# researchaccelerator-hub/distributed-crawler

Hardware: AMD Instinct MI355X
Metric: posts/sec (whole node) synthetic feed (higher is better)
Workload: dtype uint8; 1 GPU; model=telegram-crawl 1k-channels x 10k-posts per GPU (BASELINE config #2, weak-scaled), global_batch=1250000, seq_len=0, platform=telegram, parallelism=dp1, channels_per_gpu=1000, posts_per_channel=10000, chunk_posts=1250000, new_discoveries=998486, sink=pinned, pinned=True, max_comments_per_post=3

## Files before the change

### crawler_amd/ops/csrc/common.h

```cpp
#pragma once

#include <hip/hip_runtime.h>
#include <stdint.h>

#define WAVE 64
#define DEV __device__ __forceinline__

typedef unsigned int __attribute__((aligned(1))) u32_unal;
#ifndef CRAWL_NT_STORES
#define CRAWL_NT_STORES 0
#endif
DEV void nt_store_u32(unsigned char* p, unsigned v) {
#if CRAWL_NT_STORES
  __builtin_nontemporal_store(v, (u32_unal*)p);
#else
  __builtin_memcpy(p, &v, 4);
#endif
}
DEV void nt_store_u8(unsigned char* p, unsigned char v) {
#if CRAWL_NT_STORES
  __builtin_nontemporal_store(v, p);
#else
  *p = v;
#endif
}

namespace crawl {

DEV int lane_id() { return threadIdx.x & (WAVE - 1); }
DEV int wave_id() { return threadIdx.x >> 6; }


DEV bool is_ascii_letter(uint8_t c) {
  return (c >= 'a' && c <= 'z') || (c >= 'A' && c <= 'Z');
}
DEV bool is_word_char(uint8_t c) {
  return is_ascii_letter(c) || (c >= '0' && c <= '9') || c == '_';
}
DEV uint8_t to_lower(uint8_t c) {
  return (c >= 'A' && c <= 'Z') ? (c + 32) : c;
}

DEV int u16_units_of_byte(uint8_t b) {
  if (b < 0x80) return 1;
  if (b < 0xC0) return 0;
  if (b < 0xF0) return 1;
  return 2;
}

__device__ const uint8_t ESC_CLS[256] = {
    0x06, 0x06, 0x06, 0x06, 0x06, 0x06, 0x06, 0x06, 0x06, 0x02, 0x02, 0x06, 0x06, 0x02, 0x06, 0x06,
    0x06, 0x06, 0x06, 0x06, 0x06, 0x06, 0x06, 0x06, 0x06, 0x06, 0x06, 0x06, 0x06, 0x06, 0x06, 0x06,
    0x01, 0x01, 0x02, 0x01, 0x01, 0x01, 0x06, 0x01, 0x01, 0x01, 0x01, 0x01, 0x01, 0x01, 0x01, 0x01,
    0x01, 0x01, 0x01, 0x01, 0x01, 0x01, 0x01, 0x01, 0x01, 0x01, 0x01, 0x01, 0x06, 0x01, 0x06, 0x01,
    0x01, 0x01, 0x01, 0x01, 0x01, 0x01, 0x01, 0x01, 0x01, 0x01, 0x01, 0x01, 0x01, 0x01, 0x01, 0x01,
    0x01, 0x01, 0x01, 0x01, 0x01, 0x01, 0x01, 0x01, 0x01, 0x01, 0x01, 0x01, 0x02, 0x01, 0x01, 0x01,
    0x01, 0x01, 0x01, 0x01, 0x01, 0x01, 0x01, 0x01, 0x01, 0x01, 0x01, 0x01, 0x01, 0x01, 0x01, 0x01,
    0x01, 0x01, 0x01, 0x01, 0x01, 0x01, 0x01, 0x01, 0x01, 0x01, 0x01, 0x01, 0x01, 0x01, 0x01, 0x01,
    0xFF, 0x01, 0x01, 0x01, 0x01, 0x01, 0x01, 0x01, 0x01, 0x01, 0x01, 0x01, 0x01, 0x01, 0x01, 0x01,
    0x01, 0x01, 0x01, 0x01, 0x01, 0x01, 0x01, 0x01, 0x01, 0x01, 0x01, 0x01, 0x01, 0x01, 0x01, 0x01,
    0x01, 0x01, 0x01, 0x01, 0x01, 0x01, 0x01, 0x01, 0xFF, 0xFF, 0x01, 0x01, 0x01, 0x01, 0x01, 0x01,
    0x01, 0x01, 0x01, 0x01, 0x01, 0x01, 0x01, 0x01, 0x01, 0x01, 0x01, 0x01, 0x01, 0x01, 0x01, 0x01,
    0x01, 0x01, 0x01, 0x01, 0x01, 0x01, 0x01, 0x01, 0x01, 0x01, 0x01, 0x01, 0x01, 0x01, 0x01, 0x01,
    0x01, 0x01, 0x01, 0x01, 0x01, 0x01, 0x01, 0x01, 0x01, 0x01, 0x01, 0x01, 0x01, 0x01, 0x01, 0x01,
    0x01, 0x01, 0xFF, 0x01, 0x01, 0x01, 0x01, 0x01, 0x01, 0x01, 0x01, 0x01, 0x01, 0x01, 0x01, 0x01,
    0x01, 0x01, 0x01, 0x01, 0x01, 0x01, 0x01, 0x01, 0x01, 0x01, 0x01, 0x01, 0x01, 0x01, 0x01, 0x01,
};

DEV int escape_len_at(const uint8_t* s, int n, int p) {
  uint8_t c = s[p];
  uint8_t v = ESC_CLS[c];
  if (v != 0xFF) return v;
  if (c == 0xE2) {
    if (p + 2 < n && s[p + 1] == 0x80 &&
        (s[p + 2] == 0xA8 || s[p + 2] == 0xA9))
      return 6;
    return 1;
  }
  if (c == 0x80) {
    if (p >= 1 && s[p - 1] == 0xE2 && p + 1 < n &&
        (s[p + 1] == 0xA8 || s[p + 1] == 0xA9))
      return 0;
    return 1;
  }
  if (p >= 2 && s[p - 2] == 0xE2 && s[p - 1] == 0x80) return 0;
  return 1;
}

DEV const char* HEXD() { return "0123456789abcdef"; }

DEV int escape_write_at(const uint8_t* s, int n, int p, uint8_t* out) {
  uint8_t c = s[p];
  switch (c) {
    case '"':  out[0] = '\\'; out[1] = '"';  return 2;
    case '\\': out[0] = '\\'; out[1] = '\\'; return 2;
    case '\n': out[0] = '\\'; out[1] = 'n';  return 2;
    case '\r': out[0] = '\\'; out[1] = 'r';  return 2;
    case '\t': out[0] = '\\'; out[1] = 't';  return 2;
    default: break;
  }
  if (c < 0x20 || c == '<' || c == '>' || c == '&') {
    out[0] = '\\'; out[1] = 'u'; out[2] = '0'; out[3] = '0';
    out[4] = HEXD()[c >> 4]; out[5] = HEXD()[c & 15];
    return 6;
  }
  if (c == 0xE2 && p + 2 < n && s[p + 1] == 0x80 &&
      (s[p + 2] == 0xA8 || s[p + 2] == 0xA9)) {
    out[0] = '\\'; out[1] = 'u'; out[2] = '2'; out[3] = '0'; out[4] = '2';
    out[5] = (s[p + 2] == 0xA8) ? '8' : '9';
    return 6;
  }
  if (escape_len_at(s, n, p) == 0) return 0;
  out[0] = c;
  return 1;
}


DEV int wave_prefix_excl(int v) {
  int lane = lane_id();
  for (int d = 1; d < WAVE; d <<= 1) {
    int up = __shfl_up(v, d);
    if (lane >= d) v += up;
  }
  return __shfl_up(v, 1) * (lane > 0 ? 1 : 0);
}

DEV int wave_sum(int v) {
  for (int d = WAVE / 2; d > 0; d >>= 1) v += __shfl_down(v, d);
  return __shfl(v, 0);
}


DEV int u64_dec_len(uint64_t v) {
  if (v < 10ULL) return 1;
  if (v < 100ULL) return 2;
  if (v < 1000ULL) return 3;
  if (v < 10000ULL) return 4;
  if (v < 100000ULL) return 5;
  if (v < 1000000ULL) return 6;
  if (v < 10000000ULL) return 7;
  if (v < 100000000ULL) return 8;
  if (v < 1000000000ULL) return 9;
  if (v < 10000000000ULL) return 10;
  if (v < 100000000000ULL) return 11;
  if (v < 1000000000000ULL) return 12;
  if (v < 10000000000000ULL) return 13;
  if (v < 100000000000000ULL) return 14;
  if (v < 1000000000000000ULL) return 15;
  if (v < 10000000000000000ULL) return 16;
  if (v < 100000000000000000ULL) return 17;
  if (v < 1000000000000000000ULL) return 18;
  if (v < 10000000000000000000ULL) return 19;
  return 20;
}
DEV int i64_dec_len(int64_t v) {
  return (v < 0) ? 1 + u64_dec_len((uint64_t)(-v)) : u64_dec_len((uint64_t)v);
}

DEV void rfc3339_write(uint8_t* out, int cur, long long secs) {
  long long days = secs / 86400;
  long long rem = secs % 86400;
  if (rem < 0) { rem += 86400; days -= 1; }
  int hh = (int)(rem / 3600), mm = (int)((rem % 3600) / 60),
      ss = (int)(rem % 60);
  long long z = days + 719468;
  long long era = (z >= 0 ? z : z - 146096) / 146097;
  long long doe = z - era * 146097;
  long long yoe = (doe - doe / 1460 + doe / 36524 - doe / 146096) / 365;
  long long y = yoe + era * 400;
  long long doy = doe - (365 * yoe + yoe / 4 - yoe / 100);
  long long mp = (5 * doy + 2) / 153;
  long long d = doy - (153 * mp + 2) / 5 + 1;
  long long m = mp + (mp < 10 ? 3 : -9);
  y += (m <= 2);
  int yy = (int)y, mo = (int)m, dd = (int)d;
  auto pk = [](int a, int b, int c, int e) {
    return (unsigned)a | ((unsigned)b << 8) | ((unsigned)c << 16) |
           ((unsigned)e << 24);
  };
  unsigned w0 = pk('0' + (yy / 1000) % 10, '0' + (yy / 100) % 10,
                   '0' + (yy / 10) % 10, '0' + yy % 10);
  unsigned w1 = pk('-', '0' + mo / 10, '0' + mo % 10, '-');
  unsigned w2 = pk('0' + dd / 10, '0' + dd % 10, 'T', '0' + hh / 10);
  unsigned w3 = pk('0' + hh % 10, ':', '0' + mm / 10, '0' + mm % 10);
  unsigned w4 = pk(':', '0' + ss / 10, '0' + ss % 10, 'Z');
  int lane = lane_id();
  if (lane < 5) {
    unsigned v = w0;
    if (lane == 1) v = w1;
    else if (lane == 2) v = w2;
    else if (lane == 3) v = w3;
    else if (lane == 4) v = w4;
    nt_store_u32(out + cur + 4 * lane, v);
  }
}

#define LIT(e, s)                                              \
  do {                                                         \
    if ((int)sizeof(s) - 1 <= 4)                               \
      (e).template lit_small<(int)sizeof(s) - 1>(s);           \
    else                                                       \
      (e).raw((const unsigned char*)(s), (int)sizeof(s) - 1);  \
  } while (0)

template <bool W>
struct JsonEmit {
  uint8_t* out;
  int cur;
  const uint8_t* lds;

  DEV void lds_lit(int off, int n) {
    if (W) {
      const uint8_t* s = lds + off;
      int lane = lane_id();
      int nw = n >> 2;
      for (int k = lane; k < nw; k += WAVE) {
        unsigned w;
        __builtin_memcpy(&w, s + 4 * k, 4);
        nt_store_u32(out + cur + 4 * k, w);
      }
      for (int j = (nw << 2) + lane; j < n; j += WAVE)
        nt_store_u8(out + cur + j, s[j]);
    }
    cur += n;
  }

  template <int N, int M>
  DEV void lit_small(const char (&str)[M]) {
    if (W && lane_id() == 0) {
      if (N == 1) {
        out[cur] = (unsigned char)str[0];
      } else if (N == 2) {
        unsigned short v = (unsigned short)((unsigned char)str[0] |
                                            ((unsigned char)str[1] << 8));
        __builtin_memcpy(out + cur, &v, 2);
      } else {
        unsigned v = (unsigned)(unsigned char)str[0] |
                     ((unsigned)(unsigned char)str[1] << 8) |
                     ((N > 2 ? (unsigned)(unsigned char)str[2] : 0u) << 16) |
                     ((N > 3 ? (unsigned)(unsigned char)str[3] : 0u) << 24);
        if (N == 4)
          __builtin_memcpy(out + cur, &v, 4);
        else {
          __builtin_memcpy(out + cur, &v, 2);
          out[cur + 2] = (unsigned char)str[2];
        }
      }
    }
    cur += N;
  }

  DEV void raw(const uint8_t* s, int n) {
    if (W) {
      int lane = lane_id();
      int nw = n >> 2;
      for (int k = lane; k < nw; k += WAVE) {
        unsigned w;
        __builtin_memcpy(&w, s + 4 * k, 4);
        nt_store_u32(out + cur + 4 * k, w);
      }
      for (int j = (nw << 2) + lane; j < n; j += WAVE)
        nt_store_u8(out + cur + j, s[j]);
    }
    cur += n;
  }

  static DEV bool swar_special(unsigned w) {
    unsigned hz;
    unsigned nonascii = w & 0x80808080u;
    unsigned lt20 = (w - 0x20202020u) & ~w & 0x80808080u;
    if (lt20) return true;
    hz = ((w ^ 0x22222222u) - 0x01010101u) & ~(w ^ 0x22222222u);
    hz |= ((w ^ 0x5C5C5C5Cu) - 0x01010101u) & ~(w ^ 0x5C5C5C5Cu);
    hz |= ((w ^ 0x3C3C3C3Cu) - 0x01010101u) & ~(w ^ 0x3C3C3C3Cu);
    hz |= ((w ^ 0x3E3E3E3Eu) - 0x01010101u) & ~(w ^ 0x3E3E3E3Eu);
    hz |= ((w ^ 0x26262626u) - 0x01010101u) & ~(w ^ 0x26262626u);
    if (hz & 0x80808080u) return true;
    if (nonascii) {
      unsigned e2 = ((w ^ 0xE2E2E2E2u) - 0x01010101u) & ~(w ^ 0xE2E2E2E2u);
      if (e2 & 0x80808080u) return true;
    }
    return false;
  }

  DEV void esc(const uint8_t* s, int n) {
    int lane = lane_id();
    int start = 0;
    while (start < n) {
      if (start + 4 * WAVE <= n) {
        bool risk = (start >= 1 && s[start - 1] == 0xE2) ||
                    (start >= 2 && s[start - 2] == 0xE2 &&
                     s[start - 1] == 0x80);
        if (!risk) {
          unsigned w;
          __builtin_memcpy(&w, s + start + 4 * lane, 4);
          if (__ballot(swar_special(w)) == 0) {
            if (W)
              nt_store_u32(out + cur + 4 * lane, w);
            cur += 4 * WAVE;
            start += 4 * WAVE;
            continue;
          }
        }
      }
      esc_stripe(s, n, start, lane);
      start += WAVE;
    }
  }

  DEV void esc_stripe(const uint8_t* s, int n, int start, int lane) {
    {
      int p = start + lane;
      int span = n - start;
      if (span > WAVE) span = WAVE;
      int el = (p < n) ? escape_len_at(s, n, p) : 0;
      unsigned long long dirty = __ballot(p < n && el != 1);
      if (dirty == 0) {
        if (W && p < n) nt_store_u8(out + cur + p - start, s[p]);
        cur += span;
        return;
      }
      if (W) {
        int off = wave_prefix_excl(el);
        if (p < n && el > 0) {
          escape_write_at(s, n, p, out + cur + off);
        }
      }
      cur += wave_sum(el);
    }
  }

  DEV void u64(unsigned long long v) {
    static const unsigned long long POW10[20] = {
        1ULL, 10ULL, 100ULL, 1000ULL, 10000ULL, 100000ULL, 1000000ULL,
        10000000ULL, 100000000ULL, 1000000000ULL, 10000000000ULL,
        100000000000ULL, 1000000000000ULL, 10000000000000ULL,
        100000000000000ULL, 1000000000000000ULL, 10000000000000000ULL,
        100000000000000000ULL, 1000000000000000000ULL,
        10000000000000000000ULL};
    int n = u64_dec_len(v);
    if (W) {
      int lane = lane_id();
      if (lane < n) {
        unsigned d;
        if (v <= 0xFFFFFFFFULL)
          d = ((unsigned)v / (unsigned)POW10[lane]) % 10u;
        else
          d = (unsigned)((v / POW10[lane]) % 10ULL);
        nt_store_u8(out + cur + n - 1 - lane, (uint8_t)('0' + d));
      }
    }
    cur += n;
  }
  DEV void i64(long long v) {
    if (v < 0) { LIT(*this, "-"); u64((unsigned long long)(-v)); }
    else u64((unsigned long long)v);
  }

  DEV void rfc3339(long long secs) {
    if (W) rfc3339_write(out, cur, secs);
    cur += 20;
  }
};

DEV uint64_t fnv1a64(const uint8_t* s, int n) {
  uint64_t h = 1469598103934665603ULL;
  for (int i = 0; i < n; ++i) {
    h ^= s[i];
    h *= 1099511628211ULL;
  }
  return h;
}

}
```

### crawler_amd/ops/csrc/gen_lits.py

```python
#!/usr/bin/env python3
import os
import re

SRC = os.path.join(os.path.dirname(os.path.abspath(__file__)),
                   "parse_encode.hip")
OUT = os.path.join(os.path.dirname(os.path.abspath(__file__)),
                   "tg_lits.h")


def c_unescape_len(lit: str) -> int:
    i = 0
    n = 0
    while i < len(lit):
        if lit[i] == "\\":
            i += 2
        else:
            i += 1
        n += 1
    return n


def main():
    src = open(SRC).read()
    start = src.index("DEV int emit_line")
    end = src.index("\n}", start)
    body = src[start:end]
    lits = re.findall(r'LIT\(e,\s*((?:"(?:[^"\\]|\\.)*"\s*)+)\)', body)
    strings = []
    for raw in lits:
        segs = re.findall(r'"((?:[^"\\]|\\.)*)"', raw)
        strings.append("".join(segs))
    seen = {}
    order = []
    for s in strings:
        if c_unescape_len(s) >= 5 and s not in seen:
            seen[s] = f"TGL_{len(order)}"
            order.append(s)

    lines = ["// GENERATED by gen_lits.py — do not edit by hand.",
             "// LDS literal pool for parse_encode.hip's emit_line.",
             "#pragma once", "", "namespace crawl {", ""]
    lines.append("#define TG_LIT_STRS(X) \\")
    for s in order:
        lines.append(f'  X({seen[s]}, "{s}") \\')
    lines.append("")
    lines.append("enum TgLitId {")
    lines.append("#define TG_ID(name, str) name##_id,")
    lines.append("TG_LIT_STRS(TG_ID)")
    lines.append("#undef TG_ID")
    lines.append("  TG_NLITS")
    lines.append("};")
    lines.append("")
    lines.append("constexpr int tg_lit_lens[] = {")
    lines.append("#define TG_LEN(name, str) (int)sizeof(str) - 1,")
    lines.append("TG_LIT_STRS(TG_LEN)")
    lines.append("#undef TG_LEN")
    lines.append("};")
    lines.append("""
constexpr int tg_lit_off(int id) {
  int o = 0;
  for (int k = 0; k < id; ++k) o += tg_lit_lens[k];
  return o;
}
constexpr int TG_POOL_BYTES = tg_lit_off(TG_NLITS);

template <int N> struct TgCharArr { char v[N]; };
constexpr TgCharArr<TG_POOL_BYTES> tg_make_pool() {
  TgCharArr<TG_POOL_BYTES> a{};
  int o = 0;
#define TG_CP(name, str) \\
  for (int k = 0; k < (int)sizeof(str) - 1; ++k) a.v[o++] = (str)[k];
TG_LIT_STRS(TG_CP)
#undef TG_CP
  return a;
}
__device__ constexpr TgCharArr<TG_POOL_BYTES> tg_lit_pool = tg_make_pool();

// call-site macro: emit pooled literal `name` from the LDS copy
#define TGLIT(e, name) \\
  (e).lds_lit(tg_lit_off(name##_id), tg_lit_lens[name##_id])
""")
    lines.append("}  // namespace crawl")
    open(OUT, "w").write("\n".join(lines) + "\n")
    print(f"{len(order)} pooled literals, {sum(c_unescape_len(s) for s in order)} bytes")

    def repl(m):
        segs = re.findall(r'"((?:[^"\\]|\\.)*)"', m.group(1))
        s = "".join(segs)
        if s in seen:
            return f"TGLIT(e, {seen[s]})"
        return m.group(0)

    new_body = re.sub(r'LIT\(e,\s*((?:"(?:[^"\\]|\\.)*"\s*)+)\)', repl,
                      body)
    open(SRC, "w").write(src[:start] + new_body + src[end:])
    n = len(re.findall(r"TGLIT\(", new_body))
    print(f"rewrote {n} call sites in emit_line")


if __name__ == "__main__":
    main()
```

### crawler_amd/ops/csrc/parse_encode.hip

```cpp

#include "common.h"
#include "tg_lits.h"
#include "views.h"

namespace crawl {

#define MAX_LINKS 8
#define TG_STAGE_BYTES 3968

struct BatchView {
  BatchView_FIELDS_0(VIEW_MEMBER)
  int created_len;
  BatchView_FIELDS_1(VIEW_MEMBER)
  int capture_len;
  int n;
  int skip_media;
  long min_post_date;
  BatchView_FIELDS_2(VIEW_MEMBER)
};

struct LinkOut {
  LinkOut_FIELDS(VIEW_MEMBER)
};


DEV void utf16_to_bytes(const unsigned char* s, int n, int off16, int len16,
                        int* out_start, int* out_end) {
  int lane = lane_id();
  int run = 0;
  int start = -1, end = -1;
  const int t1 = off16, t2 = off16 + len16;
  for (int base = 0; base < n; base += WAVE) {
    int p = base + lane;
    int u = (p < n) ? u16_units_of_byte(s[p]) : 0;
    int pre = run + wave_prefix_excl(u);
    bool boundary = (p < n) && u > 0;
    unsigned long long m1 = __ballot(boundary && pre == t1);
    unsigned long long m2 = __ballot(boundary && pre == t2);
    if (start < 0 && m1) start = base + __ffsll(m1) - 1;
    if (end < 0 && m2) end = base + __ffsll(m2) - 1;
    run += wave_sum(u);
    if (end >= 0) break;
  }
  if (start < 0) { *out_start = 0; *out_end = 0; return; }
  *out_start = start;
  *out_end = (end >= 0) ? end : n;
}


DEV bool is_reserved_path(const unsigned char* name, int n) {
  const char* tbl[10] = {"joinchat", "addlist", "addstickers", "addtheme",
                         "setlanguage", "share", "proxy", "socks", "login",
                         "confirm"};
  const int lens[10] = {8, 7, 11, 8, 11, 5, 5, 5, 5, 7};
  for (int k = 0; k < 10; ++k) {
    if (lens[k] != n) continue;
    bool eq = true;
    for (int j = 0; j < n; ++j) eq &= (name[j] == (unsigned char)tbl[k][j]);
    if (eq) return true;
  }
  return false;
}

DEV int match_name_at(const unsigned char* s, int hi, int q,
                      unsigned char* name, bool* reserved) {
  *reserved = false;
  if (q >= hi || !is_ascii_letter(s[q])) return 0;
  int len = 0;
  while (len < 32 && q + len < hi && is_word_char(s[q + len])) ++len;
  if (len < 5) return 0;
  for (int j = 0; j < len; ++j) name[j] = to_lower(s[q + j]);
  *reserved = is_reserved_path(name, len);
  return len;
}

DEV int find_tme(const unsigned char* s, int from, int hi, int lane) {
  for (int base = from; base + 5 <= hi; base += WAVE) {
    int p = base + lane;
    bool m = (p + 5 <= hi) && s[p] == 't' && s[p + 1] == '.' &&
             s[p + 2] == 'm' && s[p + 3] == 'e' && s[p + 4] == '/';
    unsigned long long bal = __ballot(m);
    if (bal) return base + __ffsll(bal) - 1;
  }
  return -1;
}

DEV int find_username(const unsigned char* s, int lo, int hi, int lane,
                      unsigned char* name) {
  for (int base = lo; base < hi; base += WAVE) {
    int p = base + lane;
    bool m = false;
    if (p < hi && p + 5 <= hi && is_ascii_letter(s[p])) {
      m = is_word_char(s[p + 1]) && is_word_char(s[p + 2]) &&
          is_word_char(s[p + 3]) && is_word_char(s[p + 4]);
    }
    unsigned long long bal = __ballot(m);
    if (bal) {
      int q = base + __ffsll(bal) - 1;
      int len = 0;
      while (len < 32 && q + len < hi && is_word_char(s[q + len])) ++len;
      for (int j = 0; j < len; ++j) name[j] = to_lower(s[q + j]);
      return len;
    }
  }
  return 0;
}

struct LinkList {
  unsigned char* names;
  unsigned char* lens;
  unsigned char* srcs;
  unsigned long long* hashes;
  int cnt;

  DEV void add(const unsigned char* name, int len, int src, int lane) {
    for (int k = 0; k < cnt; ++k) {
      if (lens[k] != (unsigned char)len) continue;
      bool eq = true;
      for (int j = 0; j < len; ++j) eq &= (names[k * 32 + j] == name[j]);
      if (eq) return;
    }
    if (cnt >= MAX_LINKS) return;
    if (lane == 0) {
      for (int j = 0; j < len; ++j) names[cnt * 32 + j] = name[j];
      lens[cnt] = (unsigned char)len;
      srcs[cnt] = (unsigned char)src;
      hashes[cnt] = fnv1a64(name, len);
    }
    ++cnt;
  }
};

DEV void extract_links(const BatchView& B, int i, LinkList& L, int lane) {
  int ct = B.content_type[i];
  if (ct > 6) return;
  const unsigned char* text = B.pool + B.text_off[i];
  const int tn = B.text_len[i];
  unsigned char name[32];

  const int e0 = B.ent_off[i], ec = B.ent_cnt[i];
  for (int e = e0; e < e0 + ec; ++e) {
    const int* row = B.entities + (long)e * 5;
    int etype = row[0];
    if (etype == 1) {
      const unsigned char* url = B.pool + row[3];
      int un = row[4];
      for (int from = 0;;) {
        int p = find_tme(url, from, un, lane);
        if (p < 0) break;
        bool rsv;
        int len = match_name_at(url, un, p + 5, name, &rsv);
        if (len) {
          if (!rsv) L.add(name, len, 1, lane);
          break;
        }
        from = p + 1;
      }
    } else {
      int lo, hi;
      utf16_to_bytes(text, tn, row[1], row[2], &lo, &hi);
      if (!(lo < hi && hi <= tn)) continue;
      if (etype == 0) {
        int len = find_username(text, lo, hi, lane, name);
        if (len) L.add(name, len, 0, lane);
      } else {
        for (int from = lo;;) {
          int p = find_tme(text, from, hi, lane);
          if (p < 0) break;
          bool rsv;
          int len = match_name_at(text, hi, p + 5, name, &rsv);
          if (len) {
            if (!rsv) L.add(name, len, 2, lane);
            break;
          }
          from = p + 1;
        }
      }
    }
  }

  int cursor = 0;
  int from = 0;
  while (true) {
    int p = find_tme(text, from, tn, lane);
    if (p < 0) break;
    from = p + 1;
    if (p < cursor) continue;
    bool rsv;
    int len = match_name_at(text, tn, p + 5, name, &rsv);
    if (len) {
      if (!rsv) L.add(name, len, 3, lane);
      cursor = p + 5 + len;
      from = cursor;
    }
  }
}


template <bool W>
struct Emit : JsonEmit<W> {
  DEV void qesc(const unsigned char* s, int n) {
    LIT(*this, "\"");
    this->esc(s, n);
    LIT(*this, "\"");
  }
};

struct StagedTabs {
  const unsigned char* emoji_pool;
  const int* emoji_off;
  const int* emoji_len;
  const unsigned char* created;
  const unsigned char* capture;
  const unsigned char* ctname_pool;
  const int* ctname_off;
  const int* ctname_len;
};

template <bool W, bool STAGED>
DEV int emit_line(const BatchView& B, int i, unsigned char* out,
                  LinkList& L, const unsigned char* lds_lits,
                  unsigned char* lds_stage, const StagedTabs* T) {
  const int lane = lane_id();
  Emit<W> e{};
  e.out = out;
  e.cur = 0;
  e.lds = lds_lits;
  const int c = B.channel_idx[i];
  const unsigned char* user = B.pool + B.ch_user_off[c];
  const int user_n = B.ch_user_len[c];
  const unsigned char* title = B.pool + B.ch_title_off[c];
  const int title_n = B.ch_title_len[c];
  const long pub_id = B.msg_id[i] >> 20;
  const int ct = B.content_type[i];
  const int ncom = B.com_cnt[i];
  const bool has_user = user_n > 0;
  const long chat_id_v = B.chat_id[i];
  const int media_album = B.media_album_id[i];
  const int date_v = B.date[i];
  const int views_v = B.views[i];
  const int forwards_v = B.forwards[i];
  const int ch_member_v = B.ch_member[c];
  const int ch_postcount_v = B.ch_postcount[c];
  const int ch_totalviews_v = B.ch_totalviews[c];
  const int flags_v = B.flags[i];
  const int com0_v = B.com_off[i];
  const int react0_v = B.react_off[i];
  const int reactc_v = B.react_cnt[i];
  const int poster_off_v = B.poster_off[i];
  const int poster_len_v = B.poster_len[i];
  const int text_off_v = B.text_off[i];
  const int text_len_v = B.text_len[i];
  const int aux_off_v = B.aux_off[i];
  const int aux_len_v = B.aux_len[i];
  const int ctname_off_v = B.ctname_off[ct];
  const int ctname_len_v = B.ctname_len[ct];
  const unsigned char* desc_p;
  int desc_n;
  if (ct == 0 || ct == 1 || ct == 2 || ct == 4 || ct == 14) {
    desc_p = B.pool + text_off_v;
    desc_n = text_len_v;
  } else if (ct == 3 || ct == 9 || ct == 10 || ct == 11) {
    desc_p = B.pool + aux_off_v;
    desc_n = aux_len_v;
  } else {
    desc_p = nullptr;
    desc_n = 0;
  }
  const unsigned char* poster_p = B.pool + poster_off_v;
  const int* re_src = B.react_emoji + react0_v;
  const int* rcnt_src = B.react_count + react0_v;
  const unsigned char* lnames_src = L.names;
  const unsigned char* llens_src = L.lens;
  if (STAGED) {
    int stage_o = 0;
    auto staged = [&](const unsigned char* ptr,
                      int n) -> const unsigned char* {
      unsigned char* dst = lds_stage + stage_o;
      stage_o += n;
      for (int j = lane; j < n; j += WAVE) dst[j] = ptr[j];
      return dst;
    };
    user = staged(user, user_n);
    title = staged(title, title_n);
    poster_p = staged(poster_p, poster_len_v);
    desc_p = staged(desc_p, desc_n);
    lnames_src = staged(L.names, L.cnt * 32);
    llens_src = staged(L.lens, L.cnt);
    stage_o = (stage_o + 3) & ~3;
    int* s_re = (int*)(lds_stage + stage_o);
    stage_o += reactc_v * 4;
    int* s_rc = (int*)(lds_stage + stage_o);
    stage_o += reactc_v * 4;
    for (int j = lane; j < reactc_v; j += WAVE) {
      s_re[j] = B.react_emoji[react0_v + j];
      s_rc[j] = B.react_count[react0_v + j];
    }
    re_src = s_re;
    rcnt_src = s_rc;
  }
  const unsigned char* emoji_pool_s = STAGED ? T->emoji_pool : B.emoji_pool;
  const int* emoji_off_s = STAGED ? T->emoji_off : B.emoji_off;
  const int* emoji_len_s = STAGED ? T->emoji_len : B.emoji_len;
  const unsigned char* created_s = STAGED ? T->created : B.created_str;
  const unsigned char* capture_s = STAGED ? T->capture : B.capture_str;
  const unsigned char* ctpool_s = STAGED ? T->ctname_pool : B.ctname_pool;

  auto post_link = [&]() {
    if (!has_user) { LIT(e, "\"\""); return; }
    TGLIT(e, TGL_0);
    e.esc(user, user_n);
    LIT(e, "/");
    e.i64(pub_id);
    if (media_album != 0) TGLIT(e, TGL_1);
    LIT(e, "\"");
  };

  TGLIT(e, TGL_2);
  post_link();
  TGLIT(e, TGL_3);
  e.i64(chat_id_v);
  TGLIT(e, TGL_4);
  e.i64(pub_id);
  LIT(e, "-");
  e.esc(user, user_n);
  TGLIT(e, TGL_5);
  post_link();
  TGLIT(e, TGL_6);
  e.rfc3339(date_v);
  TGLIT(e, TGL_7);
  e.raw(created_s, B.created_len);
  TGLIT(e, TGL_8);
  e.i64(views_v);
  TGLIT(e, TGL_9);
  e.i64(views_v);
  TGLIT(e, TGL_10);
  e.i64(forwards_v);
  TGLIT(e, TGL_11);
  e.i64(ncom);
  TGLIT(e, TGL_12);
  e.qesc(title, title_n);
  TGLIT(e, TGL_13);
  e.i64(chat_id_v);
  TGLIT(e, TGL_14);
  e.qesc(title, title_n);
  TGLIT(e, TGL_15);
  e.i64(ch_member_v);
  TGLIT(e, TGL_16);
  e.i64(ch_postcount_v);
  TGLIT(e, TGL_17);
  e.i64(ch_totalviews_v);
  TGLIT(e, TGL_18);
  e.esc(user, user_n);
  TGLIT(e, TGL_19);
  e.esc(user, user_n);
  TGLIT(e, TGL_20);
  e.qesc(desc_p, desc_n);
  TGLIT(e, TGL_21);
  e.raw(ctpool_s + (STAGED ? T->ctname_off[ct] : ctname_off_v),
        STAGED ? T->ctname_len[ct] : ctname_len_v);
  TGLIT(e, TGL_22);
  e.i64(forwards_v);
  TGLIT(e, TGL_23);
  e.i64(ncom);
  TGLIT(e, TGL_17);
  e.i64(views_v);
  TGLIT(e, TGL_24);
  TGLIT(e, TGL_25);
  if ((ct == 3 || ct == 8) && (flags_v & 2)) {
    LIT(e, "AgAD");
    e.i64(pub_id);
    LIT(e, "v");
  }
  TGLIT(e, TGL_26);
  {
    const int c0 = com0_v;
    for (int k = 0; k < ncom; ++k) {
      if (k) LIT(e, ",");
      const int cc = c0 + k;
      TGLIT(e, TGL_27);
      e.qesc(B.pool + B.com_text_off[cc], B.com_text_len[cc]);
      TGLIT(e, TGL_28);
      const int r0 = B.com_react_off[cc], rc = B.com_react_cnt[cc];
      for (int r = 0; r < rc; ++r) {
        if (r) LIT(e, ",");
        int em = B.react_emoji[r0 + r];
        LIT(e, "\"");
        e.raw(emoji_pool_s + emoji_off_s[em], emoji_len_s[em]);
        LIT(e, "\":");
        e.i64(B.react_count[r0 + r]);
      }
      TGLIT(e, TGL_29);
      e.i64(B.com_views[cc]);
      TGLIT(e, TGL_30);
      e.i64(B.com_replies[cc]);
      TGLIT(e, TGL_31);
      e.qesc(B.pool + B.com_handle_off[cc], B.com_handle_len[cc]);
      LIT(e, "}");
    }
  }
  TGLIT(e, TGL_32);
  {
    const int rc = reactc_v;
    for (int r = 0; r < rc; ++r) {
      if (r) LIT(e, ",");
      int em = re_src[r];
      LIT(e, "\"");
      e.raw(emoji_pool_s + emoji_off_s[em], emoji_len_s[em]);
      LIT(e, "\":");
      e.i64(rcnt_src[r]);
    }
  }
  TGLIT(e, TGL_33);
  for (int k = 0; k < L.cnt; ++k) {
    if (k) LIT(e, ",");
    LIT(e, "\"");
    e.raw(lnames_src + k * 32, llens_src[k]);
    LIT(e, "\"");
  }
  TGLIT(e, TGL_34);
  e.raw(capture_s, B.capture_len);
  TGLIT(e, TGL_35);
  e.qesc(poster_p, poster_len_v);
  LIT(e, "}\n");
  return e.cur;
}


DEV LinkList links_of(const LinkOut& LO, int i, int cnt) {
  return LinkList{LO.name + (size_t)i * MAX_LINKS * 32,
                  LO.name_len + (size_t)i * MAX_LINKS,
                  LO.src + (size_t)i * MAX_LINKS,
                  LO.hash + (size_t)i * MAX_LINKS, cnt};
}

__global__ void __launch_bounds__(256, 6)
measure_extract_kernel(BatchView B, LinkOut LO, int* __restrict__ line_len) {
  __shared__ unsigned char s_lits[TG_POOL_BYTES];
  __shared__ unsigned char s_ln[4][MAX_LINKS * 32];
  __shared__ unsigned char s_ll[4][MAX_LINKS];
  __shared__ unsigned char s_ls[4][MAX_LINKS];
  __shared__ unsigned long long s_lh[4][MAX_LINKS];
  for (int t = threadIdx.x; t < TG_POOL_BYTES; t += blockDim.x)
    s_lits[t] = (unsigned char)tg_lit_pool.v[t];
  __syncthreads();
  const int lane = lane_id();
  const int wave = wave_id();
  const int waves_per_grid = gridDim.x * 4;
  for (int i = blockIdx.x * 4 + wave; i < B.n; i += waves_per_grid) {
    if ((long)B.date[i] < B.min_post_date) {
      if (lane == 0) { line_len[i] = 0; LO.cnt[i] = 0; }
      continue;
    }
    LinkList L{&s_ln[wave][0], &s_ll[wave][0], &s_ls[wave][0],
               &s_lh[wave][0], 0};
    extract_links(B, i, L, lane);
    int len = emit_line<false, false>(B, i, nullptr, L, s_lits,
                                     nullptr, nullptr);
    const int nb = L.cnt * 32;
    unsigned char* gname = LO.name + (size_t)i * MAX_LINKS * 32;
    for (int j = lane; j < nb; j += WAVE) gname[j] = s_ln[wave][j];
    if (lane < L.cnt) {
      LO.name_len[(size_t)i * MAX_LINKS + lane] = s_ll[wave][lane];
      LO.src[(size_t)i * MAX_LINKS + lane] = s_ls[wave][lane];
      LO.hash[(size_t)i * MAX_LINKS + lane] = s_lh[wave][lane];
    }
    if (lane == 0) {
      line_len[i] = len;
      LO.cnt[i] = L.cnt;
    }
  }
}

__global__ void __launch_bounds__(256, 4)
write_kernel(BatchView B, LinkOut LO, const long* __restrict__ line_off,
             const int* __restrict__ line_len, unsigned char* __restrict__ out) {
  __shared__ unsigned char s_lits[TG_POOL_BYTES];
  for (int t = threadIdx.x; t < TG_POOL_BYTES; t += blockDim.x)
    s_lits[t] = (unsigned char)tg_lit_pool.v[t];
  __syncthreads();
  const int lane = lane_id();
  const int wave = wave_id();
  const int waves_per_grid = gridDim.x * 4;
  for (int i = blockIdx.x * 4 + wave; i < B.n; i += waves_per_grid) {
    if (line_len[i] == 0) continue;
    LinkList L = links_of(LO, i, LO.cnt[i]);
    emit_line<true, false>(B, i, out + line_off[i], L, s_lits, nullptr,
                           nullptr);
  }
}

#define TG_EMOJI_POOL_CAP 512
#define TG_EMOJI_CAP 64
#define TG_TS_CAP 64
#define TG_CTNAME_POOL_CAP 512
#define TG_CTNAME_CAP 32

__global__ void __launch_bounds__(256, 4)
write_staged_kernel(BatchView B, LinkOut LO, const long* __restrict__ line_off,
                    const int* __restrict__ line_len,
                    unsigned char* __restrict__ out,
                    int n_emoji, int emoji_pool_bytes,
                    int n_ctnames, int ctname_pool_bytes) {
  __shared__ unsigned char s_lits[TG_POOL_BYTES];
  __shared__ unsigned char s_stage[4][TG_STAGE_BYTES];
  __shared__ unsigned char s_emoji_pool[TG_EMOJI_POOL_CAP];
  __shared__ int s_emoji_off[TG_EMOJI_CAP];
  __shared__ int s_emoji_len[TG_EMOJI_CAP];
  __shared__ unsigned char s_created[TG_TS_CAP];
  __shared__ unsigned char s_capture[TG_TS_CAP];
  __shared__ unsigned char s_ctpool[TG_CTNAME_POOL_CAP];
  __shared__ int s_ctoff[TG_CTNAME_CAP];
  __shared__ int s_ctlen[TG_CTNAME_CAP];
  for (int t = threadIdx.x; t < TG_POOL_BYTES; t += blockDim.x)
    s_lits[t] = (unsigned char)tg_lit_pool.v[t];
  for (int t = threadIdx.x; t < emoji_pool_bytes; t += blockDim.x)
    s_emoji_pool[t] = B.emoji_pool[t];
  for (int t = threadIdx.x; t < n_emoji; t += blockDim.x) {
    s_emoji_off[t] = B.emoji_off[t];
    s_emoji_len[t] = B.emoji_len[t];
  }
  for (int t = threadIdx.x; t < B.created_len; t += blockDim.x)
    s_created[t] = B.created_str[t];
  for (int t = threadIdx.x; t < B.capture_len; t += blockDim.x)
    s_capture[t] = B.capture_str[t];
  for (int t = threadIdx.x; t < ctname_pool_bytes; t += blockDim.x)
    s_ctpool[t] = B.ctname_pool[t];
  for (int t = threadIdx.x; t < n_ctnames; t += blockDim.x) {
    s_ctoff[t] = B.ctname_off[t];
    s_ctlen[t] = B.ctname_len[t];
  }
  __syncthreads();
  StagedTabs T{s_emoji_pool, s_emoji_off, s_emoji_len, s_created,
               s_capture, s_ctpool, s_ctoff, s_ctlen};
  const int lane = lane_id();
  const int wave = wave_id();
  const int waves_per_grid = gridDim.x * 4;
  for (int i = blockIdx.x * 4 + wave; i < B.n; i += waves_per_grid) {
    if (line_len[i] == 0) continue;
    LinkList L = links_of(LO, i, LO.cnt[i]);
    emit_line<true, true>(B, i, out + line_off[i], L, s_lits,
                          &s_stage[wave][0], &T);
  }
}


#define LDS_LINE_BYTES 3072

DEV void copy_line(const unsigned char* src, unsigned char* dst, int n,
                   int lane);

__global__ void __launch_bounds__(256)
write_lds_kernel(BatchView B, LinkOut LO, const long* __restrict__ line_off,
                 const int* __restrict__ line_len, unsigned char* __restrict__ out) {
  __shared__ unsigned char lbuf[4][LDS_LINE_BYTES];
  __shared__ unsigned char s_lits[TG_POOL_BYTES];
  for (int t = threadIdx.x; t < TG_POOL_BYTES; t += blockDim.x)
    s_lits[t] = (unsigned char)tg_lit_pool.v[t];
  __syncthreads();
  const int lane = lane_id();
  const int wave = wave_id();
  const int waves_per_grid = gridDim.x * 4;
  for (int i = blockIdx.x * 4 + wave; i < B.n; i += waves_per_grid) {
    const int len = line_len[i];
    if (len == 0) continue;
    LinkList L = links_of(LO, i, LO.cnt[i]);
    if (len > LDS_LINE_BYTES) {
      emit_line<true, false>(B, i, out + line_off[i], L, s_lits,
                             nullptr, nullptr);
      continue;
    }
    emit_line<true, false>(B, i, &lbuf[wave][0], L, s_lits, nullptr,
                           nullptr);
    copy_line(&lbuf[wave][0], out + line_off[i], len, lane);
  }
}


__global__ void __launch_bounds__(256)
write_scratch_kernel(BatchView B, LinkOut LO, unsigned char* __restrict__ scratch,
                     long stride, int* __restrict__ line_len, int* __restrict__ overflow) {
  __shared__ unsigned char s_lits[TG_POOL_BYTES];
  for (int t = threadIdx.x; t < TG_POOL_BYTES; t += blockDim.x)
    s_lits[t] = (unsigned char)tg_lit_pool.v[t];
  __syncthreads();
  const int lane = lane_id();
  const int wave = wave_id();
  const int waves_per_grid = gridDim.x * 4;
  for (int i = blockIdx.x * 4 + wave; i < B.n; i += waves_per_grid) {
    if ((long)B.date[i] < B.min_post_date) {
      if (lane == 0) { line_len[i] = 0; LO.cnt[i] = 0; }
      continue;
    }
    LinkList L = links_of(LO, i, 0);
    extract_links(B, i, L, lane);
    int len = emit_line<true, false>(B, i, scratch + (size_t)i * stride, L,
                                     s_lits, nullptr, nullptr);
    if (lane == 0) {
      line_len[i] = len;
      LO.cnt[i] = L.cnt;
      if (len > stride) atomicMax(overflow, len);
    }
  }
}

DEV void copy_line(const unsigned char* src, unsigned char* dst, int n,
                   int lane) {
  int h = (int)((4 - ((unsigned long)(size_t)dst & 3)) & 3);
  if (h > n) h = n;
  if (lane == 0)
    for (int j = 0; j < h; ++j) dst[j] = src[j];
  const unsigned char* s = src + h;
  unsigned char* d = dst + h;
  int rem = n - h;
  int nw = rem >> 2;
  int sh = (int)((unsigned long)(size_t)s & 3);
  const unsigned int* sw = (const unsigned int*)(s - sh);
  for (int k = lane; k < nw; k += WAVE) {
    unsigned int w0 = sw[k];
    unsigned int v;
    if (sh) {
      unsigned int w1 = sw[k + 1];
      v = (unsigned int)((((unsigned long long)w1 << 32) | w0) >> (8 * sh));
    } else {
      v = w0;
    }
    ((unsigned int*)d)[k] = v;
  }
  if (lane == 0)
    for (int j = h + (nw << 2); j < n; ++j) dst[j] = src[j];
}

__global__ void __launch_bounds__(256)
compact_kernel(const unsigned char* scratch, long stride,
               const long* line_off, const int* line_len,
               unsigned char* out, int n) {
  const int lane = lane_id();
  const int wave = wave_id();
  const int waves_per_grid = gridDim.x * 4;
  for (int i = blockIdx.x * 4 + wave; i < n; i += waves_per_grid) {
    int len = line_len[i];
    if (len == 0) continue;
    copy_line(scratch + (size_t)i * stride, out + line_off[i], len, lane);
  }
}

}


namespace crawl {

static BatchView make_view(void** p, const long* s) {
  BatchView V;
  int k = 0;
  BatchView_FIELDS(VIEW_UNPACK)
  V.n = (int)s[0];
  V.skip_media = (int)s[1];
  V.min_post_date = s[2];
  V.created_len = (int)s[3];
  V.capture_len = (int)s[4];
  return V;
}

static LinkOut make_links(void** p) {
  LinkOut V;
  int k = 0;
  LinkOut_FIELDS(VIEW_UNPACK)
  return V;
}

struct Views {
  BatchView B;
  LinkOut LO;
};

static Views make_views(void** batch_ptrs, const long* scalars,
                        void** link_ptrs) {
  return {make_view(batch_ptrs, scalars), make_links(link_ptrs)};
// ... 77 lines not shown
```

### crawler_amd/ops/csrc/tg_lits.h

```cpp
#pragma once

namespace crawl {

#define TG_LIT_STRS(X) \
  X(TGL_0, "\"https://t.me/") \
  X(TGL_1, "?single") \
  X(TGL_2, "{\"post_link\":") \
  X(TGL_3, ",\"channel_id\":\"") \
  X(TGL_4, "\",\"post_uid\":\"") \
  X(TGL_5, "\",\"url\":") \
  X(TGL_6, ",\"published_at\":\"") \
  X(TGL_7, "\",\"created_at\":\"") \
  X(TGL_8, "\",\"language_code\":\"\",\"engagement\":") \
  X(TGL_9, ",\"view_count\":") \
  X(TGL_10, ",\"like_count\":0,\"share_count\":") \
  X(TGL_11, ",\"comment_count\":") \
  X(TGL_12, ",\"crawl_label\":\"\",\"list_ids\":null,\"channel_name\":") \
  X(TGL_13, ",\"search_terms\":null,\"search_term_ids\":null,\"project_ids\":null,\"exercise_ids\":null,\"label_data\":null,\"labels_metadata\":null,\"project_labeled_post_ids\":null,\"labeler_ids\":null,\"all_labels\":null,\"label_ids\":null,\"is_ad\":false,\"transcript_text\":\"\",\"image_text\":\"\",\"video_length\":null,\"is_verified\":null,\"channel_data\":{\"channel_id\":\"") \
  X(TGL_14, "\",\"channel_name\":") \
  X(TGL_15, ",\"channel_description\":\"\",\"channel_profile_image\":\"\",\"channel_engagement_data\":{\"follower_count\":") \
  X(TGL_16, ",\"following_count\":0,\"like_count\":0,\"post_count\":") \
  X(TGL_17, ",\"views_count\":") \
  X(TGL_18, ",\"comment_count\":0,\"share_count\":0},\"channel_url_external\":\"https://t.me/c/") \
  X(TGL_19, "\",\"channel_url\":\"https://t.me/c/") \
  X(TGL_20, "\",\"country_code\":\"\",\"published_at\":\"0001-01-01T00:00:00Z\"},\"platform_name\":\"Telegram\",\"shared_id\":null,\"quoted_id\":null,\"replied_id\":null,\"ai_label\":null,\"root_post_id\":null,\"engagement_steps_count\":0,\"ocr_data\":null,\"performance_scores\":{\"likes\":null,\"shares\":null,\"comments\":null,\"views\":0},\"has_embed_media\":null,\"description\":") \
  X(TGL_21, ",\"repost_channel_data\":null,\"post_type\":[\"") \
  X(TGL_22, "\"],\"inner_link\":{},\"post_title\":null,\"media_data\":{\"document_name\":\"\"},\"is_reply\":null,\"ad_fields\":null,\"likes_count\":0,\"shares_count\":") \
  X(TGL_23, ",\"comments_count\":") \
  X(TGL_24, ",\"searchable_text\":\"\",\"all_text\":\"\",\"contrast_agent_project_ids\":null,\"agent_ids\":null,\"segment_ids\":null,\"thumb_url\":\"") \
  X(TGL_25, "\",\"media_url\":\"") \
  X(TGL_26, "\",\"comments\":[") \
  X(TGL_27, "{\"text\":") \
  X(TGL_28, ",\"reactions\":{") \
  X(TGL_29, "},\"view_count\":") \
  X(TGL_30, ",\"reply_count\":") \
  X(TGL_31, ",\"handle\":") \
  X(TGL_32, "],\"reactions\":{") \
  X(TGL_33, "},\"outlinks\":[") \
  X(TGL_34, "],\"capture_time\":\"") \
  X(TGL_35, "\",\"handle\":") \

enum TgLitId {
#define TG_ID(name, str) name##_id,
TG_LIT_STRS(TG_ID)
#undef TG_ID
  TG_NLITS
};

constexpr int tg_lit_lens[] = {
#define TG_LEN(name, str) (int)sizeof(str) - 1,
TG_LIT_STRS(TG_LEN)
#undef TG_LEN
};

constexpr int tg_lit_off(int id) {
  int o = 0;
  for (int k = 0; k < id; ++k) o += tg_lit_lens[k];
  return o;
}
constexpr int TG_POOL_BYTES = tg_lit_off(TG_NLITS);

template <int N> struct TgCharArr { char v[N]; };
constexpr TgCharArr<TG_POOL_BYTES> tg_make_pool() {
  TgCharArr<TG_POOL_BYTES> a{};
  int o = 0;
#define TG_CP(name, str) \
  for (int k = 0; k < (int)sizeof(str) - 1; ++k) a.v[o++] = (str)[k];
TG_LIT_STRS(TG_CP)
#undef TG_CP
  return a;
}
__device__ constexpr TgCharArr<TG_POOL_BYTES> tg_lit_pool = tg_make_pool();

#define TGLIT(e, name) \
  (e).lds_lit(tg_lit_off(name##_id), tg_lit_lens[name##_id])

}
```

Baseline: 27.89 million posts/s.

## Measure line lengths lane-serially per tile and fold literal offsets at compile time

The measure pass now processes tiles of 64 posts per wave. Link extraction stays wave-cooperative per post and records link counts and name lengths in an LDS tile; then each lane measures its own post's JSON length serially, using a SWAR fast path for escaping. Lookup tables (escape classes, hex digits, powers of ten) become arithmetic, and literal offsets become template constants so no runtime offset walk is needed. It also hoists the per-thread name buffer into shared memory and fixes the channel name to fall back to the title. The aim is to stop wasting most lanes of a wave on scalar measuring work, at the cost of lane divergence and longer serial loops per lane.

Result: no change. 28.01 million posts/s (median of 6 runs) (+0.4%).

```diff
diff --git a/crawler_amd/ops/csrc/common.h b/crawler_amd/ops/csrc/common.h
--- a/crawler_amd/ops/csrc/common.h
+++ b/crawler_amd/ops/csrc/common.h
@@ -5,6 +5,8 @@
 
 #define WAVE 64
 #define DEV __device__ __forceinline__
+#define NO_VECTORIZE \
+  _Pragma("clang loop vectorize(disable) interleave(disable)")
 
 typedef unsigned int __attribute__((aligned(1))) u32_unal;
 #ifndef CRAWL_NT_STORES
@@ -48,28 +50,17 @@
   return 2;
 }
 
-__device__ const uint8_t ESC_CLS[256] = {
-    0x06, 0x06, 0x06, 0x06, 0x06, 0x06, 0x06, 0x06, 0x06, 0x02, 0x02, 0x06, 0x06, 0x02, 0x06, 0x06,
-    0x06, 0x06, 0x06, 0x06, 0x06, 0x06, 0x06, 0x06, 0x06, 0x06, 0x06, 0x06, 0x06, 0x06, 0x06, 0x06,
-    0x01, 0x01, 0x02, 0x01, 0x01, 0x01, 0x06, 0x01, 0x01, 0x01, 0x01, 0x01, 0x01, 0x01, 0x01, 0x01,
-    0x01, 0x01, 0x01, 0x01, 0x01, 0x01, 0x01, 0x01, 0x01, 0x01, 0x01, 0x01, 0x06, 0x01, 0x06, 0x01,
-    0x01, 0x01, 0x01, 0x01, 0x01, 0x01, 0x01, 0x01, 0x01, 0x01, 0x01, 0x01, 0x01, 0x01, 0x01, 0x01,
-    0x01, 0x01, 0x01, 0x01, 0x01, 0x01, 0x01, 0x01, 0x01, 0x01, 0x01, 0x01, 0x02, 0x01, 0x01, 0x01,
-    0x01, 0x01, 0x01, 0x01, 0x01, 0x01, 0x01, 0x01, 0x01, 0x01, 0x01, 0x01, 0x01, 0x01, 0x01, 0x01,
-    0x01, 0x01, 0x01, 0x01, 0x01, 0x01, 0x01, 0x01, 0x01, 0x01, 0x01, 0x01, 0x01, 0x01, 0x01, 0x01,
-    0xFF, 0x01, 0x01, 0x01, 0x01, 0x01, 0x01, 0x01, 0x01, 0x01, 0x01, 0x01, 0x01, 0x01, 0x01, 0x01,
-    0x01, 0x01, 0x01, 0x01, 0x01, 0x01, 0x01, 0x01, 0x01, 0x01, 0x01, 0x01, 0x01, 0x01, 0x01, 0x01,
-    0x01, 0x01, 0x01, 0x01, 0x01, 0x01, 0x01, 0x01, 0xFF, 0xFF, 0x01, 0x01, 0x01, 0x01, 0x01, 0x01,
-    0x01, 0x01, 0x01, 0x01, 0x01, 0x01, 0x01, 0x01, 0x01, 0x01, 0x01, 0x01, 0x01, 0x01, 0x01, 0x01,
-    0x01, 0x01, 0x01, 0x01, 0x01, 0x01, 0x01, 0x01, 0x01, 0x01, 0x01, 0x01, 0x01, 0x01, 0x01, 0x01,
-    0x01, 0x01, 0x01, 0x01, 0x01, 0x01, 0x01, 0x01, 0x01, 0x01, 0x01, 0x01, 0x01, 0x01, 0x01, 0x01,
-    0x01, 0x01, 0xFF, 0x01, 0x01, 0x01, 0x01, 0x01, 0x01, 0x01, 0x01, 0x01, 0x01, 0x01, 0x01, 0x01,
-    0x01, 0x01, 0x01, 0x01, 0x01, 0x01, 0x01, 0x01, 0x01, 0x01, 0x01, 0x01, 0x01, 0x01, 0x01, 0x01,
-};
+DEV int esc_class(uint8_t c) {
+  if (c < 0x20) return (c == '\t' || c == '\n' || c == '\r') ? 2 : 6;
+  if (c == '"' || c == '\\') return 2;
+  if (c == '<' || c == '>' || c == '&') return 6;
+  if (c == 0xE2 || c == 0x80 || c == 0xA8 || c == 0xA9) return 0xFF;
+  return 1;
+}
 
 DEV int escape_len_at(const uint8_t* s, int n, int p) {
   uint8_t c = s[p];
-  uint8_t v = ESC_CLS[c];
+  int v = esc_class(c);
   if (v != 0xFF) return v;
   if (c == 0xE2) {
     if (p + 2 < n && s[p + 1] == 0x80 &&
@@ -87,7 +78,9 @@
   return 1;
 }
 
-DEV const char* HEXD() { return "0123456789abcdef"; }
+DEV uint8_t hex_digit(unsigned d) {
+  return (uint8_t)(d < 10 ? '0' + d : 'a' + (d - 10));
+}
 
 DEV int escape_write_at(const uint8_t* s, int n, int p, uint8_t* out) {
   uint8_t c = s[p];
@@ -101,7 +94,7 @@
   }
   if (c < 0x20 || c == '<' || c == '>' || c == '&') {
     out[0] = '\\'; out[1] = 'u'; out[2] = '0'; out[3] = '0';
-    out[4] = HEXD()[c >> 4]; out[5] = HEXD()[c & 15];
+    out[4] = hex_digit(c >> 4); out[5] = hex_digit(c & 15);
     return 6;
   }
   if (c == 0xE2 && p + 2 < n && s[p + 1] == 0x80 &&
@@ -155,6 +148,33 @@
 }
 DEV int i64_dec_len(int64_t v) {
   return (v < 0) ? 1 + u64_dec_len((uint64_t)(-v)) : u64_dec_len((uint64_t)v);
+}
+DEV int u32_dec_len_lane(unsigned x) {
+  return 1 + (x >= 10u) + (x >= 100u) + (x >= 1000u) + (x >= 10000u) +
+         (x >= 100000u) + (x >= 1000000u) + (x >= 10000000u) +
+         (x >= 100000000u) + (x >= 1000000000u);
+}
+DEV int u64_dec_len_lane(uint64_t v) {
+  if (v <= 0xFFFFFFFFULL) return u32_dec_len_lane((unsigned)v);
+  uint64_t hi = v / 1000000000ULL;
+  if (hi <= 0xFFFFFFFFULL) return 9 + u32_dec_len_lane((unsigned)hi);
+  return 19 + (hi >= 10000000000ULL);
+}
+
+DEV unsigned pow10_u32(int k) {
+  unsigned p = (k & 1) ? 5u : 1u;
+  if (k & 2) p *= 25u;
+  if (k & 4) p *= 625u;
+  if (k & 8) p *= 390625u;
+  return p << k;
+}
+DEV uint64_t pow10_u64(int k) {
+  uint64_t p = (k & 1) ? 5ULL : 1ULL;
+  if (k & 2) p *= 25ULL;
+  if (k & 4) p *= 625ULL;
+  if (k & 8) p *= 390625ULL;
+  if (k & 16) p *= 152587890625ULL;
+  return p << k;
 }
 
 DEV void rfc3339_write(uint8_t* out, int cur, long long secs) {
@@ -203,8 +223,9 @@
       (e).raw((const unsigned char*)(s), (int)sizeof(s) - 1);  \
   } while (0)
 
-template <bool W>
+template <bool W, bool LANE_SERIAL = false>
 struct JsonEmit {
+  static_assert(!(W && LANE_SERIAL), "the lane-serial walk only measures");
   uint8_t* out;
   int cur;
   const uint8_t* lds;
@@ -214,11 +235,13 @@
       const uint8_t* s = lds + off;
       int lane = lane_id();
       int nw = n >> 2;
+      NO_VECTORIZE
       for (int k = lane; k < nw; k += WAVE) {
         unsigned w;
         __builtin_memcpy(&w, s + 4 * k, 4);
         nt_store_u32(out + cur + 4 * k, w);
       }
+      NO_VECTORIZE
       for (int j = (nw << 2) + lane; j < n; j += WAVE)
         nt_store_u8(out + cur + j, s[j]);
     }
@@ -254,11 +277,13 @@
     if (W) {
       int lane = lane_id();
       int nw = n >> 2;
+      NO_VECTORIZE
       for (int k = lane; k < nw; k += WAVE) {
         unsigned w;
         __builtin_memcpy(&w, s + 4 * k, 4);
         nt_store_u32(out + cur + 4 * k, w);
       }
+      NO_VECTORIZE
       for (int j = (nw << 2) + lane; j < n; j += WAVE)
         nt_store_u8(out + cur + j, s[j]);
     }
@@ -284,6 +309,35 @@
   }
 
   DEV void esc(const uint8_t* s, int n) {
+    if constexpr (LANE_SERIAL)
+      esc_lane(s, n);
+    else
+      esc_wave(s, n);
+  }
+
+  DEV void esc_lane(const uint8_t* s, int n) {
+    int p = 0;
+    unsigned c1 = 0, c2 = 0;
+    while (p < n) {
+      bool open = c1 == 0xE2u || (c2 == 0xE2u && c1 == 0x80u);
+      if (!open && p + 4 <= n) {
+        unsigned w;
+        __builtin_memcpy(&w, s + p, 4);
+        if (!swar_special(w)) {
+          cur += 4;
+          p += 4;
+          c1 = c2 = 0;
+          continue;
+        }
+      }
+      cur += escape_len_at(s, n, p);
+      c2 = c1;
+      c1 = s[p];
+      ++p;
+    }
+  }
+
+  DEV void esc_wave(const uint8_t* s, int n) {
     int lane = lane_id();
     int start = 0;
     while (start < n) {
@@ -331,22 +385,15 @@
   }
 
   DEV void u64(unsigned long long v) {
-    static const unsigned long long POW10[20] = {
-        1ULL, 10ULL, 100ULL, 1000ULL, 10000ULL, 100000ULL, 1000000ULL,
-        10000000ULL, 100000000ULL, 1000000000ULL, 10000000000ULL,
-        100000000000ULL, 1000000000000ULL, 10000000000000ULL,
-        100000000000000ULL, 1000000000000000ULL, 10000000000000000ULL,
-        100000000000000000ULL, 1000000000000000000ULL,
-        10000000000000000000ULL};
-    int n = u64_dec_len(v);
+    int n = LANE_SERIAL ? u64_dec_len_lane(v) : u64_dec_len(v);
     if (W) {
       int lane = lane_id();
       if (lane < n) {
         unsigned d;
         if (v <= 0xFFFFFFFFULL)
-          d = ((unsigned)v / (unsigned)POW10[lane]) % 10u;
+          d = ((unsigned)v / pow10_u32(lane)) % 10u;
         else
-          d = (unsigned)((v / POW10[lane]) % 10ULL);
+          d = (unsigned)((v / pow10_u64(lane)) % 10ULL);
         nt_store_u8(out + cur + n - 1 - lane, (uint8_t)('0' + d));
       }
     }
diff --git a/crawler_amd/ops/csrc/gen_lits.py b/crawler_amd/ops/csrc/gen_lits.py
--- a/crawler_amd/ops/csrc/gen_lits.py
+++ b/crawler_amd/ops/csrc/gen_lits.py
@@ -76,9 +76,18 @@
 }
 __device__ constexpr TgCharArr<TG_POOL_BYTES> tg_lit_pool = tg_make_pool();
 
+// Offset and length of literal ID as constants of a type: a plain call
+// of tg_lit_off() at the use site is only folded if the inliner takes
+// it, and in emit_line it did not (a real call, and a walk over
+// tg_lit_lens, per literal per line).
+template <int ID> struct TgLitAt {
+  static constexpr int off = tg_lit_off(ID);
+  static constexpr int len = tg_lit_lens[ID];
+};
+
 // call-site macro: emit pooled literal `name` from the LDS copy
 #define TGLIT(e, name) \\
-  (e).lds_lit(tg_lit_off(name##_id), tg_lit_lens[name##_id])
+  (e).lds_lit(TgLitAt<name##_id>::off, TgLitAt<name##_id>::len)
 """)
     lines.append("}  // namespace crawl")
     open(OUT, "w").write("\n".join(lines) + "\n")
diff --git a/crawler_amd/ops/csrc/parse_encode.hip b/crawler_amd/ops/csrc/parse_encode.hip
--- a/crawler_amd/ops/csrc/parse_encode.hip
+++ b/crawler_amd/ops/csrc/parse_encode.hip
@@ -62,6 +62,11 @@
   return false;
 }
 
+DEV void store_name(unsigned char* name, const unsigned char* s, int len) {
+  if (lane_id() == 0)
+    for (int j = 0; j < len; ++j) name[j] = to_lower(s[j]);
+}
+
 DEV int match_name_at(const unsigned char* s, int hi, int q,
                       unsigned char* name, bool* reserved) {
   *reserved = false;
@@ -69,7 +74,7 @@
   int len = 0;
   while (len < 32 && q + len < hi && is_word_char(s[q + len])) ++len;
   if (len < 5) return 0;
-  for (int j = 0; j < len; ++j) name[j] = to_lower(s[q + j]);
+  store_name(name, s + q, len);
   *reserved = is_reserved_path(name, len);
   return len;
 }
@@ -99,7 +104,7 @@
       int q = base + __ffsll(bal) - 1;
       int len = 0;
       while (len < 32 && q + len < hi && is_word_char(s[q + len])) ++len;
-      for (int j = 0; j < len; ++j) name[j] = to_lower(s[q + j]);
+      store_name(name, s + q, len);
       return len;
     }
   }
@@ -131,12 +136,12 @@
   }
 };
 
-DEV void extract_links(const BatchView& B, int i, LinkList& L, int lane) {
+DEV void extract_links(const BatchView& B, int i, LinkList& L, int lane,
+                       unsigned char* name) {
   int ct = B.content_type[i];
   if (ct > 6) return;
   const unsigned char* text = B.pool + B.text_off[i];
   const int tn = B.text_len[i];
-  unsigned char name[32];
 
   const int e0 = B.ent_off[i], ec = B.ent_cnt[i];
   for (int e = e0; e < e0 + ec; ++e) {
@@ -197,8 +202,8 @@
 }
 
 
-template <bool W>
-struct Emit : JsonEmit<W> {
+template <bool W, bool LANE_SERIAL>
+struct Emit : JsonEmit<W, LANE_SERIAL> {
   DEV void qesc(const unsigned char* s, int n) {
     LIT(*this, "\"");
     this->esc(s, n);
@@ -217,12 +222,12 @@
   const int* ctname_len;
 };
 
-template <bool W, bool STAGED>
+template <bool W, bool STAGED, bool LANE_SERIAL = false>
 DEV int emit_line(const BatchView& B, int i, unsigned char* out,
                   LinkList& L, const unsigned char* lds_lits,
                   unsigned char* lds_stage, const StagedTabs* T) {
   const int lane = lane_id();
-  Emit<W> e{};
+  Emit<W, LANE_SERIAL> e{};
   e.out = out;
   e.cur = 0;
   e.lds = lds_lits;
@@ -278,6 +283,7 @@
                       int n) -> const unsigned char* {
       unsigned char* dst = lds_stage + stage_o;
       stage_o += n;
+      NO_VECTORIZE
       for (int j = lane; j < n; j += WAVE) dst[j] = ptr[j];
       return dst;
     };
@@ -292,6 +298,7 @@
     stage_o += reactc_v * 4;
     int* s_rc = (int*)(lds_stage + stage_o);
     stage_o += reactc_v * 4;
+    NO_VECTORIZE
     for (int j = lane; j < reactc_v; j += WAVE) {
       s_re[j] = B.react_emoji[react0_v + j];
       s_rc[j] = B.react_count[react0_v + j];
@@ -299,6 +306,8 @@
     re_src = s_re;
     rcnt_src = s_rc;
   }
+  const unsigned char* cname = has_user ? user : title;
+  const int cname_n = has_user ? user_n : title_n;
   const unsigned char* emoji_pool_s = STAGED ? T->emoji_pool : B.emoji_pool;
   const int* emoji_off_s = STAGED ? T->emoji_off : B.emoji_off;
   const int* emoji_len_s = STAGED ? T->emoji_len : B.emoji_len;
@@ -323,7 +332,7 @@
   TGLIT(e, TGL_4);
   e.i64(pub_id);
   LIT(e, "-");
-  e.esc(user, user_n);
+  e.esc(cname, cname_n);
   TGLIT(e, TGL_5);
   post_link();
   TGLIT(e, TGL_6);
@@ -351,9 +360,9 @@
   TGLIT(e, TGL_17);
   e.i64(ch_totalviews_v);
   TGLIT(e, TGL_18);
-  e.esc(user, user_n);
+  e.esc(cname, cname_n);
   TGLIT(e, TGL_19);
-  e.esc(user, user_n);
+  e.esc(cname, cname_n);
   TGLIT(e, TGL_20);
   e.qesc(desc_p, desc_n);
   TGLIT(e, TGL_21);
@@ -434,41 +443,58 @@
                   LO.hash + (size_t)i * MAX_LINKS, cnt};
 }
 
+#define TILE_ROW (1 + MAX_LINKS)
+
 __global__ void __launch_bounds__(256, 6)
 measure_extract_kernel(BatchView B, LinkOut LO, int* __restrict__ line_len) {
-  __shared__ unsigned char s_lits[TG_POOL_BYTES];
   __shared__ unsigned char s_ln[4][MAX_LINKS * 32];
   __shared__ unsigned char s_ll[4][MAX_LINKS];
   __shared__ unsigned char s_ls[4][MAX_LINKS];
   __shared__ unsigned long long s_lh[4][MAX_LINKS];
-  for (int t = threadIdx.x; t < TG_POOL_BYTES; t += blockDim.x)
-    s_lits[t] = (unsigned char)tg_lit_pool.v[t];
-  __syncthreads();
+  __shared__ unsigned char s_name[4][32];
+  __shared__ unsigned char s_tile[4][WAVE * TILE_ROW];
   const int lane = lane_id();
   const int wave = wave_id();
   const int waves_per_grid = gridDim.x * 4;
-  for (int i = blockIdx.x * 4 + wave; i < B.n; i += waves_per_grid) {
-    if ((long)B.date[i] < B.min_post_date) {
-      if (lane == 0) { line_len[i] = 0; LO.cnt[i] = 0; }
-      continue;
-    }
-    LinkList L{&s_ln[wave][0], &s_ll[wave][0], &s_ls[wave][0],
-               &s_lh[wave][0], 0};
-    extract_links(B, i, L, lane);
-    int len = emit_line<false, false>(B, i, nullptr, L, s_lits,
-                                     nullptr, nullptr);
-    const int nb = L.cnt * 32;
-    unsigned char* gname = LO.name + (size_t)i * MAX_LINKS * 32;
-    for (int j = lane; j < nb; j += WAVE) gname[j] = s_ln[wave][j];
-    if (lane < L.cnt) {
-      LO.name_len[(size_t)i * MAX_LINKS + lane] = s_ll[wave][lane];
-      LO.src[(size_t)i * MAX_LINKS + lane] = s_ls[wave][lane];
-      LO.hash[(size_t)i * MAX_LINKS + lane] = s_lh[wave][lane];
-    }
-    if (lane == 0) {
+  const int tiles = (B.n + WAVE - 1) / WAVE;
+  for (int t = blockIdx.x * 4 + wave; t < tiles; t += waves_per_grid) {
+    const int base = t * WAVE;
+    const int posts = (B.n - base < WAVE) ? B.n - base : WAVE;
+    for (int j = 0; j < posts; ++j) {
+      const int i = base + j;
+      unsigned char* row = &s_tile[wave][j * TILE_ROW];
+      if ((long)B.date[i] < B.min_post_date) continue;
+      LinkList L{&s_ln[wave][0], &s_ll[wave][0], &s_ls[wave][0],
+                 &s_lh[wave][0], 0};
+      extract_links(B, i, L, lane, &s_name[wave][0]);
+      const int nb = L.cnt * 32;
+      unsigned char* gname = LO.name + (size_t)i * MAX_LINKS * 32;
+      for (int k = lane; k < nb; k += WAVE) gname[k] = s_ln[wave][k];
+      if (lane < L.cnt) {
+        LO.name_len[(size_t)i * MAX_LINKS + lane] = s_ll[wave][lane];
+        LO.src[(size_t)i * MAX_LINKS + lane] = s_ls[wave][lane];
+        LO.hash[(size_t)i * MAX_LINKS + lane] = s_lh[wave][lane];
+        row[1 + lane] = s_ll[wave][lane];
+      }
+      if (lane == 0) row[0] = (unsigned char)L.cnt;
+    }
+    __builtin_amdgcn_fence(__ATOMIC_ACQ_REL, "wavefront");
+    __builtin_amdgcn_wave_barrier();
+    const int i = base + lane;
+    if (i < B.n) {
+      int len = 0, cnt = 0;
+      if (!((long)B.date[i] < B.min_post_date)) {
+        unsigned char* row = &s_tile[wave][lane * TILE_ROW];
+        cnt = row[0];
+        LinkList L{nullptr, row + 1, nullptr, nullptr, cnt};
+        len = emit_line<false, false, true>(B, i, nullptr, L, nullptr,
+                                            nullptr, nullptr);
+      }
       line_len[i] = len;
-      LO.cnt[i] = L.cnt;
-    }
+      LO.cnt[i] = cnt;
+    }
+    __builtin_amdgcn_fence(__ATOMIC_ACQ_REL, "wavefront");
+    __builtin_amdgcn_wave_barrier();
   }
 }
 
@@ -581,6 +607,7 @@
 write_scratch_kernel(BatchView B, LinkOut LO, unsigned char* __restrict__ scratch,
                      long stride, int* __restrict__ line_len, int* __restrict__ overflow) {
   __shared__ unsigned char s_lits[TG_POOL_BYTES];
+  __shared__ unsigned char s_name[4][32];
   for (int t = threadIdx.x; t < TG_POOL_BYTES; t += blockDim.x)
     s_lits[t] = (unsigned char)tg_lit_pool.v[t];
   __syncthreads();
@@ -593,7 +620,7 @@
       continue;
     }
     LinkList L = links_of(LO, i, 0);
-    extract_links(B, i, L, lane);
+    extract_links(B, i, L, lane, &s_name[wave][0]);
     int len = emit_line<true, false>(B, i, scratch + (size_t)i * stride, L,
                                      s_lits, nullptr, nullptr);
     if (lane == 0) {
diff --git a/crawler_amd/ops/csrc/tg_lits.h b/crawler_amd/ops/csrc/tg_lits.h
--- a/crawler_amd/ops/csrc/tg_lits.h
+++ b/crawler_amd/ops/csrc/tg_lits.h
@@ -72,7 +72,12 @@
 }
 __device__ constexpr TgCharArr<TG_POOL_BYTES> tg_lit_pool = tg_make_pool();
 
+template <int ID> struct TgLitAt {
+  static constexpr int off = tg_lit_off(ID);
+  static constexpr int len = tg_lit_lens[ID];
+};
+
 #define TGLIT(e, name) \
-  (e).lds_lit(tg_lit_off(name##_id), tg_lit_lens[name##_id])
+  (e).lds_lit(TgLitAt<name##_id>::off, TgLitAt<name##_id>::len)
 
 }
```
